# RobotLocomotion/pytorch-dense-correspondence

Hardware: NVIDIA H100
Metric: image-pairs/s (640x480, D=3) fwd+loss+bwd (higher is better)
Workload: dtype f32 (bf16x3 split on the wgmma tensor cores, fp32 accumulate)

## Files before the change

### pytorch-dense-correspondence_b200/csrc/conv_tc.cu

```cuda
#include <cuda.h>
#include <algorithm>
#include <cstdlib>
#include <cstring>
#include <functional>
#include <mutex>
#include <unordered_map>

#include "conv.cuh"
#include "conv_tc.cuh"

namespace ddn {

constexpr int TC_BLOCK_K = 64;
constexpr int TC_CONSUMERS = 256;
constexpr int TC_THREADS = TC_CONSUMERS + 32;
constexpr int TC_PRODUCER_WARP = TC_CONSUMERS / 32;
constexpr int TC_WIDE_THREADS = TC_CONSUMERS + 128;
constexpr int TC_A_BYTES = 128 * TC_BLOCK_K * 2;

__device__ __forceinline__ uint32_t smem_u32(const void* p) { return (uint32_t)__cvta_generic_to_shared(p); }

__device__ __forceinline__ void mbar_init(uint32_t bar, uint32_t count) {
  asm volatile("mbarrier.init.shared::cta.b64 [%0], %1;" ::"r"(bar), "r"(count));
}
// ... 91 lines not shown
        "wgmma.mma_async.sync.aligned.m64n128k16.f32.bf16.bf16 {"
        "%0, %1, %2, %3, %4, %5, %6, %7, %8, %9, %10, %11, %12, %13, %14, %15, "
        "%16, %17, %18, %19, %20, %21, %22, %23, %24, %25, %26, %27, %28, %29, %30, %31, "
        "%32, %33, %34, %35, %36, %37, %38, %39, %40, %41, %42, %43, %44, %45, %46, %47, "
        "%48, %49, %50, %51, %52, %53, %54, %55, %56, %57, %58, %59, %60, %61, %62, %63"
        "}, %64, %65, p, 1, 1, %67, %67;\n}\n"
        : "+f"(d[0]), "+f"(d[1]), "+f"(d[2]), "+f"(d[3]), "+f"(d[4]), "+f"(d[5]), "+f"(d[6]), "+f"(d[7]),
          "+f"(d[8]), "+f"(d[9]), "+f"(d[10]), "+f"(d[11]), "+f"(d[12]), "+f"(d[13]), "+f"(d[14]), "+f"(d[15]),
          "+f"(d[16]), "+f"(d[17]), "+f"(d[18]), "+f"(d[19]), "+f"(d[20]), "+f"(d[21]), "+f"(d[22]), "+f"(d[23]),
          "+f"(d[24]), "+f"(d[25]), "+f"(d[26]), "+f"(d[27]), "+f"(d[28]), "+f"(d[29]), "+f"(d[30]), "+f"(d[31]),
          "+f"(d[32]), "+f"(d[33]), "+f"(d[34]), "+f"(d[35]), "+f"(d[36]), "+f"(d[37]), "+f"(d[38]), "+f"(d[39]),
          "+f"(d[40]), "+f"(d[41]), "+f"(d[42]), "+f"(d[43]), "+f"(d[44]), "+f"(d[45]), "+f"(d[46]), "+f"(d[47]),
          "+f"(d[48]), "+f"(d[49]), "+f"(d[50]), "+f"(d[51]), "+f"(d[52]), "+f"(d[53]), "+f"(d[54]), "+f"(d[55]),
          "+f"(d[56]), "+f"(d[57]), "+f"(d[58]), "+f"(d[59]), "+f"(d[60]), "+f"(d[61]), "+f"(d[62]), "+f"(d[63])
        : "l"(a), "l"(b), "r"(scale_d), "n"(TRANS));
  }
};

template <int N, int TRANS, int NPROD>
__device__ __forceinline__ void mma_k16(float (&d)[N / 2], uint64_t a_hi, uint64_t a_lo, uint64_t b_hi, uint64_t b_lo, int accumulate) {
  if (NPROD == 3) {
    Wgmma<N>::template mma<TRANS>(d, a_hi, b_lo, accumulate);
    Wgmma<N>::template mma<TRANS>(d, a_lo, b_hi, 1);
    Wgmma<N>::template mma<TRANS>(d, a_hi, b_hi, 1);
  } else {
    Wgmma<N>::template mma<TRANS>(d, a_hi, b_hi, accumulate);
  }
}
template <int N, int TRANS, int NPROD>
__device__ __forceinline__ void mma_k16_x(float (&d)[N / 2], float (&x)[N / 2], uint64_t a_hi, uint64_t a_lo, uint64_t b_hi, uint64_t b_lo,
                                          int accumulate) {
  if (NPROD == 3) {
    Wgmma<N>::template mma<TRANS>(x, a_hi, b_lo, accumulate);
    Wgmma<N>::template mma<TRANS>(x, a_lo, b_hi, 1);
  }
  Wgmma<N>::template mma<TRANS>(d, a_hi, b_hi, accumulate);
}
template <int K>
__device__ __forceinline__ void add_cross(float (&d)[K], const float (&x)[K]) {
#pragma unroll
  for (int i = 0; i < K; ++i) d[i] += x[i];
}
template <int N, int K>
__device__ __forceinline__ float (&acc_cols(float (&d)[K]))[N / 2] {
  static_assert(N / 2 <= K, "accumulator too narrow");
  return *reinterpret_cast<float(*)[N / 2]>(&d[0]);
}

constexpr int EPI_ROWS = 4;
constexpr int EPI_STRIDE = 40;
constexpr int EPI_WARP_FLOATS = 16 * EPI_STRIDE;

template <int K>
__device__ __forceinline__ void stage_chunk(const float (&acc)[K], int c, float* st, int lane, float4 (&v)[EPI_ROWS]) {
  const int r = lane >> 2, q = (lane & 3) * 2;
#pragma unroll
  for (int jj = 0; jj < 4; ++jj) {
    const int j = 4 * c + jj;
    *reinterpret_cast<float2*>(st + r * EPI_STRIDE + 8 * jj + q) = make_float2(acc[4 * j], acc[4 * j + 1]);
    *reinterpret_cast<float2*>(st + (r + 8) * EPI_STRIDE + 8 * jj + q) = make_float2(acc[4 * j + 2], acc[4 * j + 3]);
  }
  __syncwarp();
  const int ga = lane >> 3, gb = lane & 7;
#pragma unroll
  for (int i = 0; i < EPI_ROWS; ++i) v[i] = *reinterpret_cast<const float4*>(st + (EPI_ROWS * ga + i) * EPI_STRIDE + 4 * gb);
  __syncwarp();
}

__device__ __forceinline__ uint32_t pack_bf16x2(__nv_bfloat16 a, __nv_bfloat16 b) {
  return (uint32_t)__bfloat16_as_ushort(a) | ((uint32_t)__bfloat16_as_ushort(b) << 16);
}

template <typename P>
__device__ __forceinline__ void conv_epilogue_rows(const P& p, const float4 (&v)[EPI_ROWS], size_t off, size_t rs, int n_ok, int ch,
                                                   int C, int grp, float4& s1, float4& s2) {
  float4 adv[EPI_ROWS];
#pragma unroll
  for (int i = 0; i < EPI_ROWS; ++i)
    adv[i] = (p.addend && i < n_ok) ? __ldg(reinterpret_cast<const float4*>(p.addend + off + i * rs)) : make_float4(0.f, 0.f, 0.f, 0.f);
  if (p.ep_scale) {
    const float4 sc = __ldg(reinterpret_cast<const float4*>(p.ep_scale + ch));
    const float4 sh = __ldg(reinterpret_cast<const float4*>(p.ep_shift + ch));
#pragma unroll
    for (int i = 0; i < EPI_ROWS; ++i) {
      float4 f = make_float4(fmaf(v[i].x, sc.x, sh.x) + adv[i].x, fmaf(v[i].y, sc.y, sh.y) + adv[i].y,
                             fmaf(v[i].z, sc.z, sh.z) + adv[i].z, fmaf(v[i].w, sc.w, sh.w) + adv[i].w);
      if (p.ep_relu) { f.x = fmaxf(f.x, 0.f); f.y = fmaxf(f.y, 0.f); f.z = fmaxf(f.z, 0.f); f.w = fmaxf(f.w, 0.f); }
      if (i < n_ok) {
        if (p.out) *reinterpret_cast<float4*>(p.out + off + i * rs) = f;
        if (p.out_hi) {
          const __nv_bfloat16 h0 = __float2bfloat16_rn(f.x), h1 = __float2bfloat16_rn(f.y), h2 = __float2bfloat16_rn(f.z), h3 = __float2bfloat16_rn(f.w);
          *reinterpret_cast<uint2*>(p.out_hi + off + i * rs) = make_uint2(pack_bf16x2(h0, h1), pack_bf16x2(h2, h3));
          if (p.out_lo)
            *reinterpret_cast<uint2*>(p.out_lo + off + i * rs) =
                make_uint2(pack_bf16x2(__float2bfloat16_rn(f.x - __bfloat162float(h0)), __float2bfloat16_rn(f.y - __bfloat162float(h1))),
                           pack_bf16x2(__float2bfloat16_rn(f.z - __bfloat162float(h2)), __float2bfloat16_rn(f.w - __bfloat162float(h3))));
        }
      }
    }
  } else if (p.bst.fin.a.acc) {
    float4 rw[EPI_ROWS];
    uint2 yh[EPI_ROWS];
#pragma unroll
    for (int i = 0; i < EPI_ROWS; ++i) {
      rw[i] = i < n_ok ? __ldg(reinterpret_cast<const float4*>(p.bst.raw + off + i * rs)) : make_float4(0.f, 0.f, 0.f, 0.f);
      if (p.bst.y_hi) yh[i] = i < n_ok ? __ldg(reinterpret_cast<const uint2*>(p.bst.y_hi + off + i * rs)) : make_uint2(0u, 0u);
    }
    const float4 mu = __ldg(reinterpret_cast<const float4*>(p.bst.mean + (size_t)grp * C + ch));
    const float4 is = __ldg(reinterpret_cast<const float4*>(p.bst.invstd + (size_t)grp * C + ch));
    float4 scl = make_float4(0.f, 0.f, 0.f, 0.f), be = scl;
    if (!p.bst.y_hi && p.bst.relu) {
      const float4 gm = __ldg(reinterpret_cast<const float4*>(p.bst.gamma + ch));
      be = __ldg(reinterpret_cast<const float4*>(p.bst.beta + ch));
      scl = make_float4(gm.x * is.x, gm.y * is.y, gm.z * is.z, gm.w * is.w);
    }
// ... 39 lines not shown
    s2.z += __shfl_xor_sync(0xffffffffu, s2.z, off); s2.w += __shfl_xor_sync(0xffffffffu, s2.w, off);
  }
}

__device__ __forceinline__ void named_barrier(int id, int threads) { asm volatile("bar.sync %0, %1;" ::"r"(id), "r"(threads) : "memory"); }

struct TcConvParams {
  float* out;
  const float* addend;
  int N, H, W, Cin, Cout;
  int taps_w;
  int dil;
  int stride;
  int tiles_h, tiles_w;
  int n_sub;
  int n_co;
  int full_items, tail_split, total_items;
  int imgs_per_group;
  BnFwdFinal fin;
  TcBwdStats bst;
  const float* ep_scale; const float* ep_shift; int ep_relu;
  __nv_bfloat16* out_hi; __nv_bfloat16* out_lo;
};

constexpr int TC_SUB_H = 4, TC_SUB_W = 16;
constexpr int TC_SUB_BYTES = 64 * 128;

struct TcItem { int sp, co0, width; };
__device__ __forceinline__ TcItem tc_item(const TcConvParams& p, int idx, int block_n) {
  int tile = idx, piece = 0, width = block_n;
  if (idx >= p.full_items) {
    const int j = idx - p.full_items;
    tile = p.full_items + j / p.tail_split;
    piece = j - (j / p.tail_split) * p.tail_split;
    width = block_n / p.tail_split;
  }
  TcItem it;
  it.sp = tile / p.n_co;
  it.co0 = (tile - it.sp * p.n_co) * block_n + piece * width;
  it.width = width;
  return it;
}
struct TcSub { int n, h0, w0; bool valid; };
__device__ __forceinline__ TcSub tc_sub(const TcConvParams& p, int st) {
  TcSub s;
  s.valid = st < p.n_sub;
  const int tw = st % p.tiles_w; const int t = st / p.tiles_w;
  const int th = t % p.tiles_h;
  s.n = s.valid ? t / p.tiles_h : p.N;
  s.h0 = th * TC_SUB_H; s.w0 = tw * TC_SUB_W;
  return s;
}

template <int W, int BLOCK_N, int NPROD, int STAGES>
__device__ __forceinline__ void conv_tc_mainloop(float (&acc)[W / 2], float (&accx)[W / 2], int num_kb, uint32_t& g, const uint64_t* full_bar,
                                                 const uint64_t* empty_bar, const uint8_t* smem, int wg, int lane) {
  constexpr int NSPLIT = NPROD == 3 ? 2 : 1;
  constexpr int A_BYTES = 128 * TC_BLOCK_K * 2;
  constexpr int B_BYTES = BLOCK_N * TC_BLOCK_K * 2;
  constexpr int STAGE_BYTES = NSPLIT * (A_BYTES + B_BYTES);
  for (int kb = 0; kb < num_kb; ++kb, ++g) {
    const int s = g % STAGES;
    mbar_wait(smem_u32(&full_bar[s]), (g / STAGES) & 1);
    wgmma_fence();
    const uint32_t stg = smem_u32(smem + (size_t)s * STAGE_BYTES);
    const uint64_t a_hi = gmma_desc_k(stg + wg * TC_SUB_BYTES), a_lo = gmma_desc_k(stg + A_BYTES + wg * TC_SUB_BYTES);
    const uint64_t b_hi = gmma_desc_k(stg + NSPLIT * A_BYTES), b_lo = gmma_desc_k(stg + 2 * A_BYTES + B_BYTES);
#pragma unroll
    for (int k = 0; k < TC_BLOCK_K / 16; ++k) {
      const uint64_t adv = (uint64_t)((k * 32) >> 4);
      mma_k16_x<W, 0, NPROD>(acc, accx, a_hi + adv, a_lo + adv, b_hi + adv, b_lo + adv, (kb | k) != 0);
    }
    wgmma_commit();
    wgmma_wait<1>();
    if (kb > 0 && lane == 0) mbar_arrive(smem_u32(&empty_bar[(g - 1) % STAGES]));
  }
  wgmma_wait<0>();
  fence_acc(acc);
  if (NPROD == 3) { fence_acc(accx); add_cross(acc, accx); }
  if (lane == 0) mbar_arrive(smem_u32(&empty_bar[(g - 1) % STAGES]));
}

template <int BLOCK_N, int NPROD>
__global__ void __launch_bounds__(TC_WIDE_THREADS, 1)
conv_tc_kernel(const __grid_constant__ CUtensorMap tm_a_hi, const __grid_constant__ CUtensorMap tm_a_lo,
               const __grid_constant__ CUtensorMap tm_b_hi, const __grid_constant__ CUtensorMap tm_b_lo,
               const __grid_constant__ CUtensorMap tm_bt_hi, const __grid_constant__ CUtensorMap tm_bt_lo,
               const TcConvParams p) {
  constexpr int NSPLIT = NPROD == 3 ? 2 : 1;
  constexpr int A_BYTES = 128 * TC_BLOCK_K * 2;
  constexpr int B_BYTES = BLOCK_N * TC_BLOCK_K * 2;
  constexpr int STAGE_BYTES = NSPLIT * (A_BYTES + B_BYTES);
  constexpr int STAGES = (192 * 1024) / STAGE_BYTES >= 8 ? 8 : (192 * 1024) / STAGE_BYTES;
  static_assert(STAGES >= 2, "pipeline needs at least two stages");

  extern __shared__ __align__(1024) uint8_t smem_raw[];
  uint8_t* smem = reinterpret_cast<uint8_t*>((reinterpret_cast<uintptr_t>(smem_raw) + 1023) & ~uintptr_t(1023));
  __shared__ __align__(8) uint64_t full_bar[STAGES];
  __shared__ __align__(8) uint64_t empty_bar[STAGES];
  __shared__ int s_last;
  __shared__ __align__(16) float s_stage[TC_CONSUMERS / 32][EPI_WARP_FLOATS];
  __shared__ __align__(16) float s_part[2][2][4][BLOCK_N];

  pdl_trigger();
  const int warp = __shfl_sync(0xffffffffu, threadIdx.x >> 5, 0), lane = threadIdx.x & 31;
  const int cin_chunks = p.Cin / TC_BLOCK_K;
  const int num_kb = p.taps_w * p.taps_w * cin_chunks;
  const int half = p.taps_w >> 1;

  if (threadIdx.x == 0) {
    for (int s = 0; s < STAGES; ++s) { mbar_init(smem_u32(&full_bar[s]), 1); mbar_init(smem_u32(&empty_bar[s]), TC_CONSUMERS / 32); }
    fence_barrier_init();
    tma_prefetch_desc(&tm_a_hi); tma_prefetch_desc(&tm_b_hi); tma_prefetch_desc(&tm_bt_hi);
    if (NSPLIT == 2) { tma_prefetch_desc(&tm_a_lo); tma_prefetch_desc(&tm_b_lo); tma_prefetch_desc(&tm_bt_lo); }
  }
  __syncthreads();
  pdl_wait();

  if (warp >= TC_PRODUCER_WARP) {
    setmaxnreg_dec<40>();
    if (warp == TC_PRODUCER_WARP && lane == 0) {
      uint32_t g = 0;
      for (int idx = blockIdx.x; idx < p.total_items; idx += gridDim.x) {
        const TcItem it = tc_item(p, idx, BLOCK_N);
// ... 231 lines not shown
        ++g;
      }
      wgmma_wait<0>();
      fence_acc(acc);
      if (NPROD == 3) { fence_acc(accx); add_cross(acc, accx); }
      if (lane == 0) mbar_arrive(smem_u32(&empty_bar[(g - 1) % SLOTS]));

      const size_t pix0 = ((size_t)n * p.H + h0 + EPI_ROWS * (ga & 1)) * p.W + (w0 + 8 * wg + 2 * w + (ga >> 1));
      const size_t row_stride = (size_t)p.W * 64;
      const int grp = n / p.imgs_per_group;
#pragma unroll
      for (int c = 0; c < 2; ++c) {
        float4 v[EPI_ROWS];
        stage_chunk(acc, c, st, lane, v);
        float4 s1 = make_float4(0.f, 0.f, 0.f, 0.f), s2 = s1;
        conv_epilogue_rows(p, v, pix0 * 64 + gb * 4 + c * 32, row_stride, EPI_ROWS, c * 32 + gb * 4, 64, grp, s1, s2);
        if (stats || bstats) {
          colsum_lane_groups(s1, s2);
          if (ga == 0) {
            *reinterpret_cast<float4*>(&s_part[0][warp][c * 32 + gb * 4]) = s1;
            *reinterpret_cast<float4*>(&s_part[1][warp][c * 32 + gb * 4]) = s2;
          }
        }
      }
      if (stats || bstats) {
        named_barrier(3, TC_CONSUMERS);
        if (threadIdx.x < 128) {
          const int col = threadIdx.x & 63, k = threadIdx.x >> 6;
          float s8 = 0.f;
#pragma unroll
          for (int q = 0; q < 8; ++q) s8 += s_part[k][q][col];
          red_add_f64(sum_acc + (size_t)(grp * 2 + k) * 64 + col, (double)s8);
        }
        named_barrier(3, TC_CONSUMERS);
      }
    }
    if (bstats) {
      const bool last = bn_last_cta(p.bst.fin.a.ticket, gridDim.x, threadIdx.x == 0, &s_last, [] { named_barrier(3, TC_CONSUMERS); });
      if (last)
        for (int c = threadIdx.x; c < 64; c += TC_CONSUMERS) bn_bwd_finalize_channel(p.bst.fin, c);
    } else if (stats) {
      const bool last = bn_last_cta(p.fin.a.ticket, gridDim.x, threadIdx.x == 0, &s_last, [] { named_barrier(3, TC_CONSUMERS); });
      if (last)
        for (int c = threadIdx.x; c < 64; c += TC_CONSUMERS) bn_fwd_finalize_channel(p.fin, c);
    }
  }
}

struct TcWgradParams {
  double* dwp;
  int N, H, W, Cin, Cout;
  int taps_w, dil, stride;
  int tiles_h, tiles_w;
  int kb_per_split;
};

template <int BN, int T, int NPROD>
struct WgradShape {
  static constexpr int NSPLIT = NPROD == 3 ? 2 : 1;
  static constexpr int A_STAGE = NSPLIT * TC_A_BYTES;
  static constexpr int B_PLANE = BN * TC_BLOCK_K * 2;
  static constexpr int B_STAGE = NSPLIT * B_PLANE;
  static constexpr int SA = 2;
  static constexpr int SB_RAW = (200 * 1024 - SA * A_STAGE) / B_STAGE;
  static constexpr int SB = SB_RAW > 2 * T + 1 ? 2 * T + 1 : SB_RAW;
  static constexpr size_t SMEM = (size_t)SA * A_STAGE + (size_t)SB * B_STAGE + 1024;
};

template <int BN, int T, int NPROD>
__global__ void __launch_bounds__(TC_THREADS, 1)
wgrad_tc_kernel(const __grid_constant__ CUtensorMap tm_dy_hi, const __grid_constant__ CUtensorMap tm_dy_lo,
                const __grid_constant__ CUtensorMap tm_x_hi, const __grid_constant__ CUtensorMap tm_x_lo,
                const TcWgradParams p) {
  using S = WgradShape<BN, T, NPROD>;
  constexpr int NSPLIT = S::NSPLIT, A_STAGE = S::A_STAGE, B_PLANE = S::B_PLANE, B_STAGE = S::B_STAGE, SA = S::SA, SB = S::SB;
  static_assert(SB >= 2 * T, "B ring too small");
  static_assert(T * BN <= 192, "accumulators exceed the register budget");
  constexpr int BOX_BYTES = 64 * 128;

  extern __shared__ __align__(1024) uint8_t smem_raw[];
  uint8_t* smem = reinterpret_cast<uint8_t*>((reinterpret_cast<uintptr_t>(smem_raw) + 1023) & ~uintptr_t(1023));
  uint8_t* smem_a = smem;
  uint8_t* smem_b = smem + SA * A_STAGE;
  __shared__ __align__(8) uint64_t full_a[SA], empty_a[SA], full_b[SB], empty_b[SB];

  pdl_trigger();
  const int warp = __shfl_sync(0xffffffffu, threadIdx.x >> 5, 0), lane = threadIdx.x & 31;
  const int ci_tiles = p.Cin / BN;
  const int ci0 = (blockIdx.x % ci_tiles) * BN;
  const int tap_row = blockIdx.x / ci_tiles;
  const int co0 = blockIdx.y * 128;
  const int total_kb = p.N * p.tiles_h * p.tiles_w;
  const int kb_begin = blockIdx.z * p.kb_per_split;
  const int kb_end = min(total_kb, kb_begin + p.kb_per_split);
  const int num_kb = kb_end - kb_begin;
  const int half = p.taps_w >> 1;

  if (threadIdx.x == 0) {
    for (int s = 0; s < SA; ++s) { mbar_init(smem_u32(&full_a[s]), 1); mbar_init(smem_u32(&empty_a[s]), TC_CONSUMERS / 32); }
    for (int s = 0; s < SB; ++s) { mbar_init(smem_u32(&full_b[s]), 1); mbar_init(smem_u32(&empty_b[s]), TC_CONSUMERS / 32); }
    fence_barrier_init();
    tma_prefetch_desc(&tm_dy_hi); tma_prefetch_desc(&tm_x_hi);
    if (NSPLIT == 2) { tma_prefetch_desc(&tm_dy_lo); tma_prefetch_desc(&tm_x_lo); }
  }
  __syncthreads();
  pdl_wait();
  if (num_kb <= 0) return;

  if (warp == TC_PRODUCER_WARP) {
    if (lane == 0) {
      for (int i = 0; i < num_kb; ++i) {
        int kb = kb_begin + i;
        const int tw = kb % p.tiles_w; kb /= p.tiles_w;
        const int th = kb % p.tiles_h; const int n = kb / p.tiles_h;
        const int h0 = th * 4, w0 = tw * 16;
        const int sa = i % SA;
        mbar_wait(smem_u32(&empty_a[sa]), ((i / SA) & 1) ^ 1);
        const uint32_t bar_a = smem_u32(&full_a[sa]);
        mbar_expect_tx(bar_a, A_STAGE);
#pragma unroll
        for (int hf = 0; hf < 2; ++hf) {
          tma_load_4d(smem_u32(smem_a + sa * A_STAGE + hf * BOX_BYTES), &tm_dy_hi, bar_a, co0 + 64 * hf, w0, h0, n);
          if (NSPLIT == 2)
            tma_load_4d(smem_u32(smem_a + sa * A_STAGE + TC_A_BYTES + hf * BOX_BYTES), &tm_dy_lo, bar_a, co0 + 64 * hf, w0, h0, n);
        }
#pragma unroll
        for (int t = 0; t < T; ++t) {
          const int j = i * T + t;
          const int sb = j % SB;
          mbar_wait(smem_u32(&empty_b[sb]), ((j / SB) & 1) ^ 1);
          const int r = (T == 1) ? half : tap_row;
          const int sx = (T == 1) ? half : t;
          const int hh = h0 * p.stride + (r - half) * p.dil, ww = w0 * p.stride + (sx - half) * p.dil;
          const uint32_t bar_b = smem_u32(&full_b[sb]);
          mbar_expect_tx(bar_b, B_STAGE);
#pragma unroll
          for (int part = 0; part < BN / 64; ++part) {
            tma_load_4d(smem_u32(smem_b + sb * B_STAGE + part * BOX_BYTES), &tm_x_hi, bar_b, ci0 + 64 * part, ww, hh, n);
            if (NSPLIT == 2)
              tma_load_4d(smem_u32(smem_b + sb * B_STAGE + B_PLANE + part * BOX_BYTES), &tm_x_lo, bar_b, ci0 + 64 * part, ww, hh, n);
          }
        }
      }
    }
  } else {
    const int wg = warp >> 2, w = warp & 3;
    const bool live = co0 + 64 * wg < p.Cout;
    float acc[T][BN / 2];
    for (int i = 0; i < num_kb; ++i) {
      const int sa = i % SA;
      mbar_wait(smem_u32(&full_a[sa]), (i / SA) & 1);
      const uint32_t a_addr = smem_u32(smem_a + sa * A_STAGE + wg * BOX_BYTES);
      const uint64_t a_hi = gmma_desc(a_addr, BOX_BYTES, 1024);
      const uint64_t a_lo = gmma_desc(a_addr + TC_A_BYTES, BOX_BYTES, 1024);
      wgmma_fence();
#pragma unroll
      for (int t = 0; t < T; ++t) {
        const int j = i * T + t;
        const int sb = j % SB;
        mbar_wait(smem_u32(&full_b[sb]), (j / SB) & 1);
        const uint32_t b_addr = smem_u32(smem_b + sb * B_STAGE);
        const uint64_t b_hi = gmma_desc(b_addr, BOX_BYTES, 1024);
        const uint64_t b_lo = gmma_desc(b_addr + B_PLANE, BOX_BYTES, 1024);
        if (live) {
#pragma unroll
          for (int k = 0; k < TC_BLOCK_K / 16; ++k) {
            const uint64_t adv = (uint64_t)((k * 16 * 128) >> 4);
            mma_k16<BN, 1, NPROD>(acc[t], a_hi + adv, a_lo + adv, b_hi + adv, b_lo + adv, (i | k) != 0);
          }
        }
      }
      wgmma_commit();
      wgmma_wait<1>();
      if (i > 0 && lane == 0) {
        mbar_arrive(smem_u32(&empty_a[(i - 1) % SA]));
#pragma unroll
        for (int t = 0; t < T; ++t) mbar_arrive(smem_u32(&empty_b[((i - 1) * T + t) % SB]));
      }
    }
    wgmma_wait<0>();
#pragma unroll
    for (int t = 0; t < T; ++t) fence_acc(acc[t]);
    if (live) {
      const int co = co0 + 64 * wg + 16 * w + (lane >> 2);
      const int ci = ci0 + 2 * (lane & 3);
#pragma unroll
      for (int t = 0; t < T; ++t) {
        const int tap = (T == 1) ? 0 : tap_row * p.taps_w + t;
        double* dst = p.dwp + ((size_t)tap * p.Cout + co) * p.Cin + ci;
#pragma unroll
        for (int j = 0; j < BN / 8; ++j) {
          red_add_f64(dst + 8 * j, (double)acc[t][4 * j]); red_add_f64(dst + 8 * j + 1, (double)acc[t][4 * j + 1]);
          red_add_f64(dst + (size_t)8 * p.Cin + 8 * j, (double)acc[t][4 * j + 2]);
          red_add_f64(dst + (size_t)8 * p.Cin + 8 * j + 1, (double)acc[t][4 * j + 3]);
        }
      }
    }
  }
}

struct TcWgradHaloParams {
  double* dwp;
  int N, H, W;
  int tiles_h, tiles_w, n_tiles;
};
constexpr int WGH_CONSUMERS = 384;
constexpr int WGH_THREADS = WGH_CONSUMERS + 32;
constexpr int WGH_X_SLOT = HALO_SLOT;
constexpr int WGH_DY_BYTES = 128 * 128;
__host__ __device__ constexpr int wgh_off(int tap) { return (tap % 3) * HALO_BH + tap / 3; }

template <int NPROD>
__global__ void __launch_bounds__(WGH_THREADS, 1)
wgrad64_halo_kernel(const __grid_constant__ CUtensorMap tm_x_hi, const __grid_constant__ CUtensorMap tm_x_lo,
                    const __grid_constant__ CUtensorMap tm_dy_hi, const __grid_constant__ CUtensorMap tm_dy_lo, const TcWgradHaloParams p) {
  constexpr int NSPLIT = NPROD == 3 ? 2 : 1;
  constexpr int STAGE = NSPLIT * (WGH_X_SLOT + WGH_DY_BYTES);
  constexpr int STAGES = 2;
  extern __shared__ __align__(1024) uint8_t smem_raw[];
  uint8_t* smem = reinterpret_cast<uint8_t*>((reinterpret_cast<uintptr_t>(smem_raw) + 1023) & ~uintptr_t(1023));
  __shared__ __align__(8) uint64_t full_bar[STAGES], empty_bar[STAGES];

  pdl_trigger();
  const int warp = __shfl_sync(0xffffffffu, threadIdx.x >> 5, 0), lane = threadIdx.x & 31;
  if (threadIdx.x == 0) {
    for (int s = 0; s < STAGES; ++s) { mbar_init(smem_u32(&full_bar[s]), 1); mbar_init(smem_u32(&empty_bar[s]), WGH_CONSUMERS / 32); }
    fence_barrier_init();
    tma_prefetch_desc(&tm_x_hi); tma_prefetch_desc(&tm_dy_hi);
    if (NSPLIT == 2) { tma_prefetch_desc(&tm_x_lo); tma_prefetch_desc(&tm_dy_lo); }
  }
  __syncthreads();
  pdl_wait();
  const int my_tiles = p.n_tiles > (int)blockIdx.x ? (p.n_tiles - (int)blockIdx.x + (int)gridDim.x - 1) / (int)gridDim.x : 0;
  if (my_tiles == 0) return;

  if (warp == WGH_CONSUMERS / 32) {
    if (lane == 0) {
      int i = 0;
      for (int t = blockIdx.x; t < p.n_tiles; t += gridDim.x, ++i) {
        const int tw = t % p.tiles_w; const int q = t / p.tiles_w;
        const int th = q % p.tiles_h, n = q / p.tiles_h;
        const int h0 = th * HALO_TH, w0 = tw * HALO_TW;
        const int s = i % STAGES;
        mbar_wait(smem_u32(&empty_bar[s]), ((i / STAGES) & 1) ^ 1);
        const uint32_t bar = smem_u32(&full_bar[s]);
        mbar_expect_tx(bar, NSPLIT * (HALO_BOX_BYTES + WGH_DY_BYTES));
        uint8_t* stg = smem + (size_t)s * STAGE;
// ... 340 lines not shown
  const MapKey key = {base, C, H, W, N, TC_BLOCK_K, box_h, box_w, -2};
  {
    std::lock_guard<std::mutex> lk(g_maps_mu);
    auto it = g_maps.find(key);
    if (it != g_maps.end()) { *m = it->second; return 0; }
  }
  EncodeTiledFn enc = get_encode_fn();
  if (!enc) { set_error("cuTensorMapEncodeTiled is unavailable (driver too old?)"); return DDN_EUNSUPPORTED; }
  cuuint64_t dims[4] = {(cuuint64_t)C, (cuuint64_t)H, (cuuint64_t)W, (cuuint64_t)N};
  cuuint64_t strides[3] = {(cuuint64_t)W * C * 2, (cuuint64_t)C * 2, (cuuint64_t)H * W * C * 2};
  cuuint32_t box[4] = {(cuuint32_t)TC_BLOCK_K, (cuuint32_t)box_h, (cuuint32_t)box_w, 1};
  cuuint32_t es[4] = {1, 1, 1, 1};
  CUresult r = enc(m, CU_TENSOR_MAP_DATA_TYPE_BFLOAT16, 4, const_cast<void*>(base), dims, strides, box, es,
                   CU_TENSOR_MAP_INTERLEAVE_NONE, CU_TENSOR_MAP_SWIZZLE_128B, CU_TENSOR_MAP_L2_PROMOTION_L2_128B,
                   CU_TENSOR_MAP_FLOAT_OOB_FILL_NONE);
  if (r != CUDA_SUCCESS) { set_error("cuTensorMapEncodeTiled(halo activations) failed: %d", (int)r); return DDN_EINVAL; }
  std::lock_guard<std::mutex> lk(g_maps_mu);
  if (g_maps.size() > 8192) g_maps.clear();
  g_maps[key] = *m;
  return 0;
}
static int make_act_map_halo(CUtensorMap* m, const void* base, int N, int H, int W, int C) {
  return make_act_map_hw(m, base, N, H, W, C, HALO_BH, HALO_BW);
}
static int make_weight_map(CUtensorMap* m, const void* base, int rows, int K, int box_rows) {
  const MapKey key = {base, K, rows, 0, 0, TC_BLOCK_K, box_rows, 0, -1};
  {
    std::lock_guard<std::mutex> lk(g_maps_mu);
    auto it = g_maps.find(key);
    if (it != g_maps.end()) { *m = it->second; return 0; }
  }
  EncodeTiledFn enc = get_encode_fn();
  if (!enc) { set_error("cuTensorMapEncodeTiled is unavailable (driver too old?)"); return DDN_EUNSUPPORTED; }
  cuuint64_t dims[2] = {(cuuint64_t)K, (cuuint64_t)rows};
  cuuint64_t strides[1] = {(cuuint64_t)K * 2};
  cuuint32_t box[2] = {(cuuint32_t)TC_BLOCK_K, (cuuint32_t)box_rows};
  cuuint32_t es[2] = {1, 1};
  CUresult r = enc(m, CU_TENSOR_MAP_DATA_TYPE_BFLOAT16, 2, const_cast<void*>(base), dims, strides, box, es,
                   CU_TENSOR_MAP_INTERLEAVE_NONE, CU_TENSOR_MAP_SWIZZLE_128B, CU_TENSOR_MAP_L2_PROMOTION_L2_256B,
                   CU_TENSOR_MAP_FLOAT_OOB_FILL_NONE);
  if (r != CUDA_SUCCESS) { set_error("cuTensorMapEncodeTiled(weights) failed: %d", (int)r); return DDN_EINVAL; }
  std::lock_guard<std::mutex> lk(g_maps_mu);
  if (g_maps.size() > 8192) g_maps.clear();
  g_maps[key] = *m;
  return 0;
}

static bool tc_halo_enabled() {
  static int v = -1;
  if (v < 0) { const char* e = getenv("DDN_TC_HALO"); v = (e && e[0] == '0') ? 0 : 1; }
  return v != 0;
}

template <int BN, int T, int NPROD>
static int launch_wgrad_tc(const CUtensorMap& dy_hi, const CUtensorMap& dy_lo, const CUtensorMap& x_hi, const CUtensorMap& x_lo,
                           const TcWgradParams& p, int splits, cudaStream_t st) {
  const size_t smem = WgradShape<BN, T, NPROD>::SMEM;
  static bool configured = false;
  if (!configured) {
    DDN_CUDA(cudaFuncSetAttribute(wgrad_tc_kernel<BN, T, NPROD>, cudaFuncAttributeMaxDynamicSharedMemorySize, (int)smem));
    configured = true;
  }
  const int tap_rows = (T == 1) ? 1 : p.taps_w;
  dim3 grid((unsigned)((p.Cin / BN) * tap_rows), (unsigned)ceil_div(p.Cout, 128), (unsigned)splits);
  DDN_LAUNCH((wgrad_tc_kernel<BN, T, NPROD>), grid, TC_THREADS, smem, st, dy_hi, dy_lo, x_hi, x_lo, p);
  return 0;
}

int tc_wgrad_planes(TcPlanes x, TcPlanes dy, float* dw, int N, int H, int W, int Cin, int Cout, int k, int stride, int dil,
                    int precision, double* dwp, cudaStream_t st) {
  const int want_lo = precision == DDN_PRECISION_BF16X3;
  const int taps = k * k;
  const int Ho = H / stride, Wo = W / stride;
  if (dw) DDN_TRY(launch_fill_zero(dwp, sizeof(double) * (size_t)taps * Cout * Cin, st));
  if (tc_halo_enabled() && k == 3 && Cin == 64 && Cout == 64 && stride == 1 && dil == 1 && H % HALO_TH == 0 && W % HALO_TW == 0) {
    TcWgradHaloParams hp;
    hp.dwp = dwp; hp.N = N; hp.H = H; hp.W = W; hp.tiles_h = H / HALO_TH; hp.tiles_w = W / HALO_TW; hp.n_tiles = N * hp.tiles_h * hp.tiles_w;
    CUtensorMap mx_hi, mx_lo, md_hi, md_lo;
    DDN_TRY(make_act_map_halo(&mx_hi, x.hi, N, H, W, 64));
    DDN_TRY(make_act_map_halo(&mx_lo, want_lo ? x.lo : x.hi, N, H, W, 64));
    DDN_TRY(make_act_map_hw(&md_hi, dy.hi, N, H, W, 64, HALO_TH, HALO_TW));
    DDN_TRY(make_act_map_hw(&md_lo, want_lo ? dy.lo : dy.hi, N, H, W, 64, HALO_TH, HALO_TW));
    const int nsplit = want_lo ? 2 : 1;
    const size_t smem = (size_t)2 * nsplit * (WGH_X_SLOT + WGH_DY_BYTES) + 1024;
    const int grid = std::min(hp.n_tiles, tc_worker_sms());
    {
      ProfScope ps(PROF_CONV_WGRAD_TC, 2.0 * N * H * W * 64.0 * 9 * 64, st);
      if (want_lo) {
        static bool configured = false;
        if (!configured) { DDN_CUDA(cudaFuncSetAttribute(wgrad64_halo_kernel<3>, cudaFuncAttributeMaxDynamicSharedMemorySize, (int)smem)); configured = true; }
        DDN_LAUNCH((wgrad64_halo_kernel<3>), grid, WGH_THREADS, smem, st, mx_hi, mx_lo, md_hi, md_lo, hp);
      } else {
        static bool configured = false;
        if (!configured) { DDN_CUDA(cudaFuncSetAttribute(wgrad64_halo_kernel<1>, cudaFuncAttributeMaxDynamicSharedMemorySize, (int)smem)); configured = true; }
        DDN_LAUNCH((wgrad64_halo_kernel<1>), grid, WGH_THREADS, smem, st, mx_hi, mx_lo, md_hi, md_lo, hp);
      }
    }
    if (dw) {
      int blocks = (int)std::min<int64_t>(ceil_div((int64_t)taps * Cout * Cin, 256), 4096);
      DDN_LAUNCH(unpack_wgrad_tc_kernel, blocks, 256, 0, st, dwp, dw, Cout, Cin, taps);
    }
    return 0;
  }
  const int bn = (k == 1 && Cin % 128 == 0) ? 128 : 64;
  CUtensorMap m_dy_hi, m_dy_lo, m_x_hi, m_x_lo;
  DDN_TRY(make_act_map(&m_dy_hi, dy.hi, N, Ho, Wo, Cout));
  DDN_TRY(make_act_map(&m_dy_lo, want_lo ? dy.lo : dy.hi, N, Ho, Wo, Cout));
  DDN_TRY(make_act_map(&m_x_hi, x.hi, N, H, W, Cin, stride));
  DDN_TRY(make_act_map(&m_x_lo, want_lo ? x.lo : x.hi, N, H, W, Cin, stride));
  TcWgradParams p;
  p.dwp = dwp; p.N = N; p.H = Ho; p.W = Wo; p.Cin = Cin; p.Cout = Cout; p.taps_w = k; p.dil = dil; p.stride = stride;
  p.tiles_h = (int)ceil_div(Ho, 4); p.tiles_w = (int)ceil_div(Wo, 16);
  const int total_kb = N * p.tiles_h * p.tiles_w;
  const int ctas_xy = (Cin / bn) * (k == 3 ? 3 : 1) * (int)ceil_div(Cout, 128);
  const int sms = tc_worker_sms();
  int waves = ctas_xy > sms ? 1 : (total_kb >= 64 * (sms / ctas_xy) ? 2 : 1);
  int splits = (int)std::max<int64_t>(1, std::min<int64_t>((int64_t)waves * sms / ctas_xy, ceil_div(total_kb, 4)));
  p.kb_per_split = (int)ceil_div(total_kb, splits);
  splits = (int)ceil_div(total_kb, p.kb_per_split);
  const double fl = 2.0 * N * Ho * Wo * (double)Cout * taps * Cin;
  {
    ProfScope ps(PROF_CONV_WGRAD_TC, fl, st);
#define WG(BNV, TV)                                                                                      \
  do {                                                                                                   \
    if (want_lo) DDN_TRY((launch_wgrad_tc<BNV, TV, 3>(m_dy_hi, m_dy_lo, m_x_hi, m_x_lo, p, splits, st))); \
    else DDN_TRY((launch_wgrad_tc<BNV, TV, 1>(m_dy_hi, m_dy_lo, m_x_hi, m_x_lo, p, splits, st)));         \
  } while (0)
    if (k == 3) WG(64, 3);
    else { if (bn == 128) WG(128, 1); else WG(64, 1); }
#undef WG
  }
  if (dw) {
    int blocks = (int)std::min<int64_t>(ceil_div((int64_t)taps * Cout * Cin, 256), 4096);
    DDN_LAUNCH(unpack_wgrad_tc_kernel, blocks, 256, 0, st, dwp, dw, Cout, Cin, taps);
  }
  return 0;
}

int tc_unpack_wgrads(const TcUnpackEntry* entries, int n, const double* dwp_base, float* grads_base, cudaStream_t st) {
  for (int i0 = 0; i0 < n; i0 += TC_UNPACK_MAX) {
    TcUnpackTable t; t.n = std::min(TC_UNPACK_MAX, n - i0);
    int64_t biggest = 0;
    for (int i = 0; i < t.n; ++i) { t.e[i] = entries[i0 + i]; biggest = std::max<int64_t>(biggest, (int64_t)t.e[i].Cout * t.e[i].Cin * t.e[i].taps); }
    dim3 grid((unsigned)std::min<int64_t>(ceil_div(biggest, 256 * 4), 1024), (unsigned)t.n);
    DDN_LAUNCH(unpack_wgrad_batched_kernel, grid, 256, 0, st, dwp_base, grads_base, t);
  }
  return 0;
}

bool tc_available() { return true; }
bool tc_folded_epilogue_supported() {
  static int fold = -1;
  if (fold < 0) { const char* e = getenv("DDN_FOLD_BN"); fold = (e && e[0] == '0') ? 0 : 1; }
  return fold != 0;
}

bool tc_conv_supported(int Cin, int Cout, int k, int stride, int pad, int dil, int H, int W) {
  if (Cin % 64 || Cout % 64) return false;
  if (stride == 2) { if (dil != 1 || (H & 1) || (W & 1)) return false; }
  else if (stride != 1) return false;
  if (k == 3) return pad == dil;
  if (k == 1) return pad == 0;
  return false;
}

static const size_t kMaxWeightElems = (size_t)9 * 512 * 512;
size_t tc_weight_ws_bytes() { return 2 * align_up(kMaxWeightElems * 2, 1024) + 2048; }

int tc_split(const float* x, __nv_bfloat16* hi, __nv_bfloat16* lo, int64_t n, int precision, cudaStream_t st) {
  DDN_CHECK_ARG(n % 4 == 0, "split: element count must be a multiple of 4");
  int64_t n4 = n / 4;
  int blocks = (int)std::min<int64_t>(ceil_div(n4, 256), (int64_t)num_sms() * 8);
  DDN_LAUNCH(split_bf16_kernel, blocks, 256, 0, st, x, hi, lo, n4, precision == DDN_PRECISION_BF16X3 ? 1 : 0);
  return 0;
}

int tc_pack_weights(const float* w_oihw, __nv_bfloat16* hi, __nv_bfloat16* lo, int Cout, int Cin, int k, int dgrad, int precision,
                    cudaStream_t st) {
  const size_t wel = (size_t)Cout * Cin * k * k;
  int wblocks = (int)std::min<int64_t>(ceil_div((int64_t)wel, 256), 4096);
  DDN_LAUNCH(pack_weights_tc_kernel, wblocks, 256, 0, st, w_oihw, hi, lo, Cout, Cin, k, dgrad, precision == DDN_PRECISION_BF16X3 ? 1 : 0);
  return 0;
}
// ... 255 lines not shown
```

Before: 124.3.

## Rewrite wgrad tensor-core kernel as persistent tile scheduler with unified ring

Replaces the split-K grid of wgrad CTAs (separate A/B rings, T taps per CTA) with a persistent kernel. Each CTA walks a flattened list of (co, ci, tap, K-chunk) items and reuses the shared conv mainloop with a transposed-descriptor mode, one 8-stage ring and warp-specialised register reallocation. A host heuristic picks the chunk count so the work spreads evenly over the SMs. The epilogue now goes through shared memory so the fp64 red.add writes are coalesced, and BN=128 is used for 3x3 too. The trade-off is that dy is reloaded once per tap rather than shared across three taps, and the item/K-split balance may add atomic traffic.

```diff
diff --git a/pytorch-dense-correspondence_b200/csrc/conv_tc.cu b/pytorch-dense-correspondence_b200/csrc/conv_tc.cu
--- a/pytorch-dense-correspondence_b200/csrc/conv_tc.cu
+++ b/pytorch-dense-correspondence_b200/csrc/conv_tc.cu
@@ -167,7 +167,7 @@
 constexpr int EPI_WARP_FLOATS = 16 * EPI_STRIDE;
 
 template <int K>
-__device__ __forceinline__ void stage_chunk(const float (&acc)[K], int c, float* st, int lane, float4 (&v)[EPI_ROWS]) {
+__device__ __forceinline__ void stage_write(const float (&acc)[K], int c, float* st, int lane) {
   const int r = lane >> 2, q = (lane & 3) * 2;
 #pragma unroll
   for (int jj = 0; jj < 4; ++jj) {
@@ -176,6 +176,11 @@
     *reinterpret_cast<float2*>(st + (r + 8) * EPI_STRIDE + 8 * jj + q) = make_float2(acc[4 * j + 2], acc[4 * j + 3]);
   }
   __syncwarp();
+}
+
+template <int K>
+__device__ __forceinline__ void stage_chunk(const float (&acc)[K], int c, float* st, int lane, float4 (&v)[EPI_ROWS]) {
+  stage_write(acc, c, st, lane);
   const int ga = lane >> 3, gb = lane & 7;
 #pragma unroll
   for (int i = 0; i < EPI_ROWS; ++i) v[i] = *reinterpret_cast<const float4*>(st + (EPI_ROWS * ga + i) * EPI_STRIDE + 4 * gb);
@@ -321,24 +326,26 @@
   return s;
 }
 
-template <int W, int BLOCK_N, int NPROD, int STAGES>
+template <int W, int BLOCK_N, int NPROD, int STAGES, int TRANS = 0>
 __device__ __forceinline__ void conv_tc_mainloop(float (&acc)[W / 2], float (&accx)[W / 2], int num_kb, uint32_t& g, const uint64_t* full_bar,
                                                  const uint64_t* empty_bar, const uint8_t* smem, int wg, int lane) {
   constexpr int NSPLIT = NPROD == 3 ? 2 : 1;
   constexpr int A_BYTES = 128 * TC_BLOCK_K * 2;
   constexpr int B_BYTES = BLOCK_N * TC_BLOCK_K * 2;
   constexpr int STAGE_BYTES = NSPLIT * (A_BYTES + B_BYTES);
+  constexpr uint32_t LBO = TRANS ? TC_SUB_BYTES : 16;
+  constexpr int K_STEP = TRANS ? 16 * 128 : 32;
   for (int kb = 0; kb < num_kb; ++kb, ++g) {
     const int s = g % STAGES;
     mbar_wait(smem_u32(&full_bar[s]), (g / STAGES) & 1);
     wgmma_fence();
     const uint32_t stg = smem_u32(smem + (size_t)s * STAGE_BYTES);
-    const uint64_t a_hi = gmma_desc_k(stg + wg * TC_SUB_BYTES), a_lo = gmma_desc_k(stg + A_BYTES + wg * TC_SUB_BYTES);
-    const uint64_t b_hi = gmma_desc_k(stg + NSPLIT * A_BYTES), b_lo = gmma_desc_k(stg + 2 * A_BYTES + B_BYTES);
+    const uint64_t a_hi = gmma_desc(stg + wg * TC_SUB_BYTES, LBO, 1024), a_lo = gmma_desc(stg + A_BYTES + wg * TC_SUB_BYTES, LBO, 1024);
+    const uint64_t b_hi = gmma_desc(stg + NSPLIT * A_BYTES, LBO, 1024), b_lo = gmma_desc(stg + 2 * A_BYTES + B_BYTES, LBO, 1024);
 #pragma unroll
     for (int k = 0; k < TC_BLOCK_K / 16; ++k) {
-      const uint64_t adv = (uint64_t)((k * 32) >> 4);
-      mma_k16_x<W, 0, NPROD>(acc, accx, a_hi + adv, a_lo + adv, b_hi + adv, b_lo + adv, (kb | k) != 0);
+      const uint64_t adv = (uint64_t)((k * K_STEP) >> 4);
+      mma_k16_x<W, TRANS, NPROD>(acc, accx, a_hi + adv, a_lo + adv, b_hi + adv, b_lo + adv, (kb | k) != 0);
     }
     wgmma_commit();
     wgmma_wait<1>();
@@ -676,147 +683,109 @@
   int N, H, W, Cin, Cout;
   int taps_w, dil, stride;
   int tiles_h, tiles_w;
-  int kb_per_split;
+  int total_kb;
+  int n_co, n_ci, n_tiles;
+  int chunks;
 };
 
-template <int BN, int T, int NPROD>
-struct WgradShape {
-  static constexpr int NSPLIT = NPROD == 3 ? 2 : 1;
-  static constexpr int A_STAGE = NSPLIT * TC_A_BYTES;
-  static constexpr int B_PLANE = BN * TC_BLOCK_K * 2;
-  static constexpr int B_STAGE = NSPLIT * B_PLANE;
-  static constexpr int SA = 2;
-  static constexpr int SB_RAW = (200 * 1024 - SA * A_STAGE) / B_STAGE;
-  static constexpr int SB = SB_RAW > 2 * T + 1 ? 2 * T + 1 : SB_RAW;
-  static constexpr size_t SMEM = (size_t)SA * A_STAGE + (size_t)SB * B_STAGE + 1024;
-};
-
-template <int BN, int T, int NPROD>
-__global__ void __launch_bounds__(TC_THREADS, 1)
+struct WgradItem { int co0, ci0, tap, kb0, kb1; };
+__device__ __forceinline__ WgradItem wgrad_item(const TcWgradParams& p, int idx, int bn) {
+  const int c = idx / p.n_tiles;
+  int t = idx - c * p.n_tiles;
+  WgradItem it;
+  it.co0 = (t % p.n_co) * 128; t /= p.n_co;
+  it.ci0 = (t % p.n_ci) * bn;
+  it.tap = t / p.n_ci;
+  it.kb0 = (int)((int64_t)c * p.total_kb / p.chunks);
+  it.kb1 = (int)((int64_t)(c + 1) * p.total_kb / p.chunks);
+  return it;
+}
+
+template <int BN, int NPROD>
+__global__ void __launch_bounds__(TC_WIDE_THREADS, 1)
 wgrad_tc_kernel(const __grid_constant__ CUtensorMap tm_dy_hi, const __grid_constant__ CUtensorMap tm_dy_lo,
                 const __grid_constant__ CUtensorMap tm_x_hi, const __grid_constant__ CUtensorMap tm_x_lo,
                 const TcWgradParams p) {
-  using S = WgradShape<BN, T, NPROD>;
-  constexpr int NSPLIT = S::NSPLIT, A_STAGE = S::A_STAGE, B_PLANE = S::B_PLANE, B_STAGE = S::B_STAGE, SA = S::SA, SB = S::SB;
-  static_assert(SB >= 2 * T, "B ring too small");
-  static_assert(T * BN <= 192, "accumulators exceed the register budget");
-  constexpr int BOX_BYTES = 64 * 128;
+  constexpr int NSPLIT = NPROD == 3 ? 2 : 1;
+  constexpr int B_BYTES = BN * TC_BLOCK_K * 2;
+  constexpr int STAGE_BYTES = NSPLIT * (TC_A_BYTES + B_BYTES);
+  constexpr int STAGES = (192 * 1024) / STAGE_BYTES >= 8 ? 8 : (192 * 1024) / STAGE_BYTES;
+  static_assert(STAGES >= 2, "pipeline needs at least two stages");
 
   extern __shared__ __align__(1024) uint8_t smem_raw[];
   uint8_t* smem = reinterpret_cast<uint8_t*>((reinterpret_cast<uintptr_t>(smem_raw) + 1023) & ~uintptr_t(1023));
-  uint8_t* smem_a = smem;
-  uint8_t* smem_b = smem + SA * A_STAGE;
-  __shared__ __align__(8) uint64_t full_a[SA], empty_a[SA], full_b[SB], empty_b[SB];
+  __shared__ __align__(8) uint64_t full_bar[STAGES];
+  __shared__ __align__(8) uint64_t empty_bar[STAGES];
+  __shared__ __align__(16) float s_stage[TC_CONSUMERS / 32][EPI_WARP_FLOATS];
 
   pdl_trigger();
   const int warp = __shfl_sync(0xffffffffu, threadIdx.x >> 5, 0), lane = threadIdx.x & 31;
-  const int ci_tiles = p.Cin / BN;
-  const int ci0 = (blockIdx.x % ci_tiles) * BN;
-  const int tap_row = blockIdx.x / ci_tiles;
-  const int co0 = blockIdx.y * 128;
-  const int total_kb = p.N * p.tiles_h * p.tiles_w;
-  const int kb_begin = blockIdx.z * p.kb_per_split;
-  const int kb_end = min(total_kb, kb_begin + p.kb_per_split);
-  const int num_kb = kb_end - kb_begin;
+  const int total_items = p.chunks * p.n_tiles;
   const int half = p.taps_w >> 1;
 
   if (threadIdx.x == 0) {
-    for (int s = 0; s < SA; ++s) { mbar_init(smem_u32(&full_a[s]), 1); mbar_init(smem_u32(&empty_a[s]), TC_CONSUMERS / 32); }
-    for (int s = 0; s < SB; ++s) { mbar_init(smem_u32(&full_b[s]), 1); mbar_init(smem_u32(&empty_b[s]), TC_CONSUMERS / 32); }
+    for (int s = 0; s < STAGES; ++s) { mbar_init(smem_u32(&full_bar[s]), 1); mbar_init(smem_u32(&empty_bar[s]), TC_CONSUMERS / 32); }
     fence_barrier_init();
     tma_prefetch_desc(&tm_dy_hi); tma_prefetch_desc(&tm_x_hi);
     if (NSPLIT == 2) { tma_prefetch_desc(&tm_dy_lo); tma_prefetch_desc(&tm_x_lo); }
   }
   __syncthreads();
   pdl_wait();
-  if (num_kb <= 0) return;
-
-  if (warp == TC_PRODUCER_WARP) {
-    if (lane == 0) {
-      for (int i = 0; i < num_kb; ++i) {
-        int kb = kb_begin + i;
-        const int tw = kb % p.tiles_w; kb /= p.tiles_w;
-        const int th = kb % p.tiles_h; const int n = kb / p.tiles_h;
-        const int h0 = th * 4, w0 = tw * 16;
-        const int sa = i % SA;
-        mbar_wait(smem_u32(&empty_a[sa]), ((i / SA) & 1) ^ 1);
-        const uint32_t bar_a = smem_u32(&full_a[sa]);
-        mbar_expect_tx(bar_a, A_STAGE);
-#pragma unroll
-        for (int hf = 0; hf < 2; ++hf) {
-          tma_load_4d(smem_u32(smem_a + sa * A_STAGE + hf * BOX_BYTES), &tm_dy_hi, bar_a, co0 + 64 * hf, w0, h0, n);
-          if (NSPLIT == 2)
-            tma_load_4d(smem_u32(smem_a + sa * A_STAGE + TC_A_BYTES + hf * BOX_BYTES), &tm_dy_lo, bar_a, co0 + 64 * hf, w0, h0, n);
-        }
-#pragma unroll
-        for (int t = 0; t < T; ++t) {
-          const int j = i * T + t;
-          const int sb = j % SB;
-          mbar_wait(smem_u32(&empty_b[sb]), ((j / SB) & 1) ^ 1);
-          const int r = (T == 1) ? half : tap_row;
-          const int sx = (T == 1) ? half : t;
-          const int hh = h0 * p.stride + (r - half) * p.dil, ww = w0 * p.stride + (sx - half) * p.dil;
-          const uint32_t bar_b = smem_u32(&full_b[sb]);
-          mbar_expect_tx(bar_b, B_STAGE);
+
+  if (warp >= TC_PRODUCER_WARP) {
+    setmaxnreg_dec<40>();
+    if (warp == TC_PRODUCER_WARP && lane == 0) {
+      uint32_t g = 0;
+      for (int idx = blockIdx.x; idx < total_items; idx += gridDim.x) {
+        const WgradItem it = wgrad_item(p, idx, BN);
+        const int r = it.tap / p.taps_w, sx = it.tap - r * p.taps_w;
+        const int dh = (r - half) * p.dil, dw = (sx - half) * p.dil;
+        for (int kb = it.kb0; kb < it.kb1; ++kb, ++g) {
+          const int s = g % STAGES;
+          mbar_wait(smem_u32(&empty_bar[s]), ((g / STAGES) & 1) ^ 1);
+          const int tw = kb % p.tiles_w, q = kb / p.tiles_w;
+          const int th = q % p.tiles_h, n = q / p.tiles_h;
+          const int h0 = th * TC_SUB_H, w0 = tw * TC_SUB_W;
+          const int hh = h0 * p.stride + dh, ww = w0 * p.stride + dw;
+          uint8_t* stg = smem + (size_t)s * STAGE_BYTES;
+          const uint32_t bar = smem_u32(&full_bar[s]);
+          mbar_expect_tx(bar, STAGE_BYTES);
+#pragma unroll
+          for (int hf = 0; hf < 2; ++hf) {
+            tma_load_4d(smem_u32(stg + hf * TC_SUB_BYTES), &tm_dy_hi, bar, it.co0 + 64 * hf, w0, h0, n);
+            if (NSPLIT == 2) tma_load_4d(smem_u32(stg + TC_A_BYTES + hf * TC_SUB_BYTES), &tm_dy_lo, bar, it.co0 + 64 * hf, w0, h0, n);
+          }
 #pragma unroll
           for (int part = 0; part < BN / 64; ++part) {
-            tma_load_4d(smem_u32(smem_b + sb * B_STAGE + part * BOX_BYTES), &tm_x_hi, bar_b, ci0 + 64 * part, ww, hh, n);
+            tma_load_4d(smem_u32(stg + NSPLIT * TC_A_BYTES + part * TC_SUB_BYTES), &tm_x_hi, bar, it.ci0 + 64 * part, ww, hh, n);
             if (NSPLIT == 2)
-              tma_load_4d(smem_u32(smem_b + sb * B_STAGE + B_PLANE + part * BOX_BYTES), &tm_x_lo, bar_b, ci0 + 64 * part, ww, hh, n);
+              tma_load_4d(smem_u32(stg + 2 * TC_A_BYTES + B_BYTES + part * TC_SUB_BYTES), &tm_x_lo, bar, it.ci0 + 64 * part, ww, hh, n);
           }
         }
       }
     }
   } else {
+    setmaxnreg_inc<232>();
     const int wg = warp >> 2, w = warp & 3;
-    const bool live = co0 + 64 * wg < p.Cout;
-    float acc[T][BN / 2];
-    for (int i = 0; i < num_kb; ++i) {
-      const int sa = i % SA;
-      mbar_wait(smem_u32(&full_a[sa]), (i / SA) & 1);
-      const uint32_t a_addr = smem_u32(smem_a + sa * A_STAGE + wg * BOX_BYTES);
-      const uint64_t a_hi = gmma_desc(a_addr, BOX_BYTES, 1024);
-      const uint64_t a_lo = gmma_desc(a_addr + TC_A_BYTES, BOX_BYTES, 1024);
-      wgmma_fence();
-#pragma unroll
-      for (int t = 0; t < T; ++t) {
-        const int j = i * T + t;
-        const int sb = j % SB;
-        mbar_wait(smem_u32(&full_b[sb]), (j / SB) & 1);
-        const uint32_t b_addr = smem_u32(smem_b + sb * B_STAGE);
-        const uint64_t b_hi = gmma_desc(b_addr, BOX_BYTES, 1024);
-        const uint64_t b_lo = gmma_desc(b_addr + B_PLANE, BOX_BYTES, 1024);
-        if (live) {
-#pragma unroll
-          for (int k = 0; k < TC_BLOCK_K / 16; ++k) {
-            const uint64_t adv = (uint64_t)((k * 16 * 128) >> 4);
-            mma_k16<BN, 1, NPROD>(acc[t], a_hi + adv, a_lo + adv, b_hi + adv, b_lo + adv, (i | k) != 0);
-          }
+    float* const st = s_stage[warp];
+    float acc[BN / 2], accx[BN / 2];
+    uint32_t g = 0;
+    for (int idx = blockIdx.x; idx < total_items; idx += gridDim.x) {
+      const WgradItem it = wgrad_item(p, idx, BN);
+      if (it.co0 + 64 * wg >= p.Cout) {
+        for (int kb = it.kb0; kb < it.kb1; ++kb, ++g) {
+          mbar_wait(smem_u32(&full_bar[g % STAGES]), (g / STAGES) & 1);
+          if (lane == 0) mbar_arrive(smem_u32(&empty_bar[g % STAGES]));
         }
-      }
-      wgmma_commit();
-      wgmma_wait<1>();
-      if (i > 0 && lane == 0) {
-        mbar_arrive(smem_u32(&empty_a[(i - 1) % SA]));
-#pragma unroll
-        for (int t = 0; t < T; ++t) mbar_arrive(smem_u32(&empty_b[((i - 1) * T + t) % SB]));
-      }
-    }
-    wgmma_wait<0>();
-#pragma unroll
-    for (int t = 0; t < T; ++t) fence_acc(acc[t]);
-    if (live) {
-      const int co = co0 + 64 * wg + 16 * w + (lane >> 2);
-      const int ci = ci0 + 2 * (lane & 3);
-#pragma unroll
-      for (int t = 0; t < T; ++t) {
-        const int tap = (T == 1) ? 0 : tap_row * p.taps_w + t;
-        double* dst = p.dwp + ((size_t)tap * p.Cout + co) * p.Cin + ci;
-#pragma unroll
-        for (int j = 0; j < BN / 8; ++j) {
-          red_add_f64(dst + 8 * j, (double)acc[t][4 * j]); red_add_f64(dst + 8 * j + 1, (double)acc[t][4 * j + 1]);
-          red_add_f64(dst + (size_t)8 * p.Cin + 8 * j, (double)acc[t][4 * j + 2]);
-          red_add_f64(dst + (size_t)8 * p.Cin + 8 * j + 1, (double)acc[t][4 * j + 3]);
+      } else {
+        conv_tc_mainloop<BN, BN, NPROD, STAGES, 1>(acc, accx, it.kb1 - it.kb0, g, full_bar, empty_bar, smem, wg, lane);
+        double* const dst = p.dwp + ((size_t)it.tap * p.Cout + it.co0 + 64 * wg + 16 * w) * p.Cin + it.ci0 + lane;
+#pragma unroll
+        for (int c = 0; c < BN / 32; ++c) {
+          stage_write(acc, c, st, lane);
+#pragma unroll
+          for (int i = 0; i < 16; ++i) red_add_f64(dst + (size_t)i * p.Cin + 32 * c, (double)st[i * EPI_STRIDE + lane]);
+          __syncwarp();
         }
       }
     }
@@ -1263,19 +1232,33 @@
   return v != 0;
 }
 
-template <int BN, int T, int NPROD>
+template <int BN, int NPROD>
 static int launch_wgrad_tc(const CUtensorMap& dy_hi, const CUtensorMap& dy_lo, const CUtensorMap& x_hi, const CUtensorMap& x_lo,
-                           const TcWgradParams& p, int splits, cudaStream_t st) {
-  const size_t smem = WgradShape<BN, T, NPROD>::SMEM;
+                           const TcWgradParams& p, int workers, cudaStream_t st) {
+  constexpr int NSPLIT = NPROD == 3 ? 2 : 1;
+  constexpr int STAGE_BYTES = NSPLIT * (TC_A_BYTES + BN * TC_BLOCK_K * 2);
+  constexpr int STAGES = (192 * 1024) / STAGE_BYTES >= 8 ? 8 : (192 * 1024) / STAGE_BYTES;
+  const size_t smem = (size_t)STAGES * STAGE_BYTES + 1024;
   static bool configured = false;
   if (!configured) {
-    DDN_CUDA(cudaFuncSetAttribute(wgrad_tc_kernel<BN, T, NPROD>, cudaFuncAttributeMaxDynamicSharedMemorySize, (int)smem));
+    DDN_CUDA(cudaFuncSetAttribute(wgrad_tc_kernel<BN, NPROD>, cudaFuncAttributeMaxDynamicSharedMemorySize, (int)smem));
     configured = true;
   }
-  const int tap_rows = (T == 1) ? 1 : p.taps_w;
-  dim3 grid((unsigned)((p.Cin / BN) * tap_rows), (unsigned)ceil_div(p.Cout, 128), (unsigned)splits);
-  DDN_LAUNCH((wgrad_tc_kernel<BN, T, NPROD>), grid, TC_THREADS, smem, st, dy_hi, dy_lo, x_hi, x_lo, p);
+  DDN_LAUNCH((wgrad_tc_kernel<BN, NPROD>), workers, TC_WIDE_THREADS, smem, st, dy_hi, dy_lo, x_hi, x_lo, p);
   return 0;
+}
+
+static int tc_wgrad_chunks(int tiles, int total_kb, int workers) {
+  const double even = (double)tiles * total_kb / workers;
+  const int max_s = std::max(1, total_kb / 4);
+  int best = 1;
+  double best_span = 1e300;
+  for (int s = 1; s <= max_s; ++s) {
+    const double span = (double)ceil_div((int64_t)s * tiles, workers) * (double)ceil_div(total_kb, s);
+    if (span <= 1.02 * even) return s;
+    if (span < best_span) { best_span = span; best = s; }
+  }
+  return best;
 }
 
 int tc_wgrad_planes(TcPlanes x, TcPlanes dy, float* dw, int N, int H, int W, int Cin, int Cout, int k, int stride, int dil,
@@ -1313,7 +1296,7 @@
     }
     return 0;
   }
-  const int bn = (k == 1 && Cin % 128 == 0) ? 128 : 64;
+  const int bn = Cin % 128 == 0 ? 128 : 64;
   CUtensorMap m_dy_hi, m_dy_lo, m_x_hi, m_x_lo;
   DDN_TRY(make_act_map(&m_dy_hi, dy.hi, N, Ho, Wo, Cout));
   DDN_TRY(make_act_map(&m_dy_lo, want_lo ? dy.lo : dy.hi, N, Ho, Wo, Cout));
@@ -1321,25 +1304,19 @@
   DDN_TRY(make_act_map(&m_x_lo, want_lo ? x.lo : x.hi, N, H, W, Cin, stride));
   TcWgradParams p;
   p.dwp = dwp; p.N = N; p.H = Ho; p.W = Wo; p.Cin = Cin; p.Cout = Cout; p.taps_w = k; p.dil = dil; p.stride = stride;
-  p.tiles_h = (int)ceil_div(Ho, 4); p.tiles_w = (int)ceil_div(Wo, 16);
-  const int total_kb = N * p.tiles_h * p.tiles_w;
-  const int ctas_xy = (Cin / bn) * (k == 3 ? 3 : 1) * (int)ceil_div(Cout, 128);
+  p.tiles_h = (int)ceil_div(Ho, TC_SUB_H); p.tiles_w = (int)ceil_div(Wo, TC_SUB_W);
+  p.total_kb = N * p.tiles_h * p.tiles_w;
+  p.n_co = (int)ceil_div(Cout, 128); p.n_ci = Cin / bn; p.n_tiles = p.n_co * p.n_ci * taps;
   const int sms = tc_worker_sms();
-  int waves = ctas_xy > sms ? 1 : (total_kb >= 64 * (sms / ctas_xy) ? 2 : 1);
-  int splits = (int)std::max<int64_t>(1, std::min<int64_t>((int64_t)waves * sms / ctas_xy, ceil_div(total_kb, 4)));
-  p.kb_per_split = (int)ceil_div(total_kb, splits);
-  splits = (int)ceil_div(total_kb, p.kb_per_split);
+  p.chunks = tc_wgrad_chunks(p.n_tiles, p.total_kb, sms);
+  const int workers = std::min(p.chunks * p.n_tiles, sms);
   const double fl = 2.0 * N * Ho * Wo * (double)Cout * taps * Cin;
   {
     ProfScope ps(PROF_CONV_WGRAD_TC, fl, st);
-#define WG(BNV, TV)                                                                                      \
-  do {                                                                                                   \
-    if (want_lo) DDN_TRY((launch_wgrad_tc<BNV, TV, 3>(m_dy_hi, m_dy_lo, m_x_hi, m_x_lo, p, splits, st))); \
-    else DDN_TRY((launch_wgrad_tc<BNV, TV, 1>(m_dy_hi, m_dy_lo, m_x_hi, m_x_lo, p, splits, st)));         \
-  } while (0)
-    if (k == 3) WG(64, 3);
-    else { if (bn == 128) WG(128, 1); else WG(64, 1); }
-#undef WG
+    if (bn == 128) DDN_TRY((want_lo ? launch_wgrad_tc<128, 3>(m_dy_hi, m_dy_lo, m_x_hi, m_x_lo, p, workers, st)
+                                    : launch_wgrad_tc<128, 1>(m_dy_hi, m_dy_lo, m_x_hi, m_x_lo, p, workers, st)));
+    else DDN_TRY((want_lo ? launch_wgrad_tc<64, 3>(m_dy_hi, m_dy_lo, m_x_hi, m_x_lo, p, workers, st)
+                          : launch_wgrad_tc<64, 1>(m_dy_hi, m_dy_lo, m_x_hi, m_x_lo, p, workers, st)));
   }
   if (dw) {
     int blocks = (int)std::min<int64_t>(ceil_div((int64_t)taps * Cout * Cin, 256), 4096);
```

Result: faster. 141.8 (median of 6 runs) (+14.1%).
